# geonuklee/slam-toolkit

Measured on NVIDIA B200. Metric: orb_extract_match_stereo_frames_per_s, higher is better.
Workload: dtype u8

## Files before the change

slam-toolkit_b200/csrc/sfe_extract.cu:

```cuda
#include <cuda_fp16.h>

#include <algorithm>
#include <cmath>
#include <mutex>
#include <type_traits>

#include "sfe_extract.cuh"

namespace sfe {

__device__ __forceinline__ uint32_t ldg_word_at(const uint8_t *p) {
    const uintptr_t a = (uintptr_t)p;
    const uint32_t *w = (const uint32_t *)(a & ~(uintptr_t)3);
    return __funnelshift_r(__ldg(w), __ldg(w + 1), (uint32_t)(a & 3) * 8);
}

__device__ __forceinline__ uint32_t dp4a_u8u8(uint32_t a, uint32_t b, uint32_t c) {
    uint32_t d;
    asm("dp4a.u32.u32 %0, %1, %2, %3;" : "=r"(d) : "r"(a), "r"(b), "r"(c));
    return d;
}
__device__ __forceinline__ uint32_t dp2a_lo(uint32_t a, uint32_t b, uint32_t c) {
    uint32_t d;
    asm("dp2a.lo.u32.u32 %0, %1, %2, %3;" : "=r"(d) : "r"(a), "r"(b), "r"(c));
    return d;
}
__device__ __forceinline__ uint32_t dp2a_hi(uint32_t a, uint32_t b, uint32_t c) {
    uint32_t d;
    asm("dp2a.hi.u32.u32 %0, %1, %2, %3;" : "=r"(d) : "r"(a), "r"(b), "r"(c));
    return d;
}

__global__ void __launch_bounds__(256) realign_kernel(const uint8_t *__restrict__ src, size_t src_stride, int src_pitch,
                                                      uint8_t *__restrict__ dst, size_t dst_stride, int dst_pitch, int w, int h) {
    pdl_enter();
    const int x = (blockIdx.x * 32 + threadIdx.x) * 16, y = blockIdx.y * 8 + threadIdx.y, img = blockIdx.z;
    if (x >= dst_pitch || y >= h) return;
    const uint8_t *p = src + (size_t)img * src_stride + (size_t)y * src_pitch + x;
    uint4 v;
    if (x + 20 <= w) {
        v = make_uint4(ldg_word_at(p), ldg_word_at(p + 4), ldg_word_at(p + 8), ldg_word_at(p + 12));
    } else {
        uint32_t q[4] = {0, 0, 0, 0};
#pragma unroll
        for (int k = 0; k < 16; k++)
            if (x + k < w) q[k >> 2] |= (uint32_t)__ldg(p + k) << (8 * (k & 3));
        v = make_uint4(q[0], q[1], q[2], q[3]);
    }
    *(uint4 *)(dst + (size_t)img * dst_stride + (size_t)y * dst_pitch + x) = v;
}

constexpr int kPyrTileW = 64, kPyrTileH = 64;

struct PyrStep {
    int w, h, pitch, plane_off;
    int src_w, src_pitch, src_plane_off, src_is_input;
    int xtab_off, ytab_off;
    int src_level, box_w, box_h;
    int wide_h;
};

template <bool kTma>
__global__ void __launch_bounds__(256) pyr_resize_kernel(ImgSet S, PyrStep P, const uint2 *__restrict__ xtab,
                                                         const uint2 *__restrict__ ytab, const __grid_constant__ TmaMaps M) {
    pdl_enter();
    extern __shared__ __align__(128) uint8_t pyr_smem[];
    uint16_t *pyr_u = (uint16_t *)(pyr_smem + (kTma ? P.box_w * P.box_h : 0));
    __shared__ uint64_t bar;
    const int x0 = blockIdx.x * kPyrTileW, y0 = blockIdx.y * kPyrTileH, img = blockIdx.z, tid = threadIdx.x;
    const uint2 *yt = ytab + P.ytab_off;
    const int sy_first = __ldg(&yt[y0]).x & 0xFFFF;
    const int n_rows = (int)(__ldg(&yt[min(y0 + kPyrTileH, P.h) - 1]).x >> 16) - sy_first + 1;
    const int slot = slot_of(S, img);
    const int xa = (int)__ldg(&xtab[P.xtab_off + x0]).x & ~15;
    if (kTma && tid == 0) {
        mbar_init(&bar, 1);
        mbar_expect_tx(&bar, (uint32_t)(P.box_w * P.box_h));
        const bool set_a = img < S.split;
        const CUtensorMap *map = P.src_is_input ? (set_a ? &M.lv[0] : &M.l0b) : &M.lv[P.src_level];
        const int z = P.src_is_input ? S.in_z0 + (set_a ? img : img - S.split) : slot;
        tma_load_3d(pyr_smem, map, &bar, xa, sy_first, z);
    }
    {
        const int ox = tid & (kPyrTileW - 1);
        const uint2 xt = __ldg(&xtab[P.xtab_off + min(x0 + ox, P.w - 1)]);
        const int sx = xt.x, d1 = min(sx + 1, P.src_w - 1) - sx;
        const uint32_t w0 = xt.y & 0xFFFF, w1 = xt.y >> 16;
        if (kTma && P.wide_h) {
            const int g4 = (tid & 15) * 4, gi = P.xtab_off + min(x0 + g4, (P.w - 1) & ~3);
            const uint4 ta = __ldg((const uint4 *)&xtab[gi]), tb = __ldg((const uint4 *)&xtab[gi + 2]);
            const int o0 = (int)ta.x - xa;
            const uint32_t sh8 = (uint32_t)(o0 & 3) * 8;
            const uint32_t r1 = ta.z - ta.x, r2 = tb.x - ta.x, r3 = tb.z - ta.x;
            const uint32_t s0 = 0x10u, s1 = r1 | (r1 + 1) << 4, s2 = r2 | (r2 + 1) << 4, s3 = r3 | (r3 + 1) << 4;
            __syncthreads();
            mbar_wait(&bar, 0);
            const uint32_t *p = (const uint32_t *)pyr_smem + (tid >> 4) * (P.box_w >> 2) + (o0 >> 2);
            const int step = 16 * (P.box_w >> 2);
            for (int r = tid >> 4; r < n_rows; r += 16) {
                const uint32_t a = __funnelshift_r(p[0], p[1], sh8), b = __funnelshift_r(p[1], p[2], sh8);
                const uint32_t u0 = dp2a_lo(ta.y, __byte_perm(a, b, s0), 0) >> 4, u1 = dp2a_lo(ta.w, __byte_perm(a, b, s1), 0) >> 4;
                const uint32_t u2 = dp2a_lo(tb.y, __byte_perm(a, b, s2), 0) >> 4, u3 = dp2a_lo(tb.w, __byte_perm(a, b, s3), 0) >> 4;
                *(uint2 *)&pyr_u[r * kPyrTileW + g4] = make_uint2(u0 | u1 << 16, u2 | u3 << 16);
                p += step;
            }
        } else if (kTma) {
            __syncthreads();
            mbar_wait(&bar, 0);
            const uint8_t *p = pyr_smem + (tid >> 6) * P.box_w + (sx - xa);
            const int step = 4 * P.box_w;
            for (int r = tid >> 6; r < n_rows; r += 4) {
                pyr_u[r * kPyrTileW + ox] = (uint16_t)((p[0] * w0 + p[d1] * w1) >> 4);
                p += step;
            }
        } else {
            const uint8_t *src;
            if (P.src_is_input)
                src = img < S.split ? S.in_a + (size_t)img * S.in_stride : S.in_b + (size_t)(img - S.split) * S.in_stride;
            else
                src = S.pyr + (size_t)slot * S.pyr_stride + P.src_plane_off;
            const uint8_t *p = src + (size_t)(sy_first + (tid >> 6)) * P.src_pitch + sx;
            const int step = 4 * P.src_pitch;
            for (int r = tid >> 6; r < n_rows; r += 4) {
                pyr_u[r * kPyrTileW + ox] = (uint16_t)((__ldg(p) * w0 + __ldg(p + d1) * w1) >> 4);
                p += step;
            }
        }
    }
    __syncthreads();
    const int cg = (tid & 15) * 4, ry = tid >> 4;
    if (x0 + cg >= P.w) return;
    uint8_t *dst = S.pyr + (size_t)slot * S.pyr_stride + P.plane_off + x0 + cg;
#pragma unroll
    for (int k = 0; k < kPyrTileH / 16; k++) {
        const int oy = y0 + ry + 16 * k;
        if (oy >= P.h) break;
        const uint2 t = __ldg(&yt[oy]);
        const int r0 = (int)(t.x & 0xFFFF) - sy_first, r1 = (int)(t.x >> 16) - sy_first;
        const uint32_t b0 = t.y << 16, b1 = t.y & 0xFFFF0000u;
        const uint2 A = *(const uint2 *)&pyr_u[r0 * kPyrTileW + cg], B = *(const uint2 *)&pyr_u[r1 * kPyrTileW + cg];
        const uint32_t a[4] = {A.x & 0xFFFF, A.x >> 16, A.y & 0xFFFF, A.y >> 16};
        const uint32_t b[4] = {B.x & 0xFFFF, B.x >> 16, B.y & 0xFFFF, B.y >> 16};
        uint32_t v[4];
#pragma unroll
        for (int i = 0; i < 4; i++) v[i] = (__umulhi(b0, a[i]) + __umulhi(b1, b[i]) + 2) >> 2;
        *(uint32_t *)(dst + (size_t)oy * P.pitch) = v[0] | v[1] << 8 | v[2] << 16 | v[3] << 24;
    }
}


template <int TP>
__device__ __forceinline__ void fast_best_x2(const uint8_t *c0, const uint8_t *c1, int &best0, int &best1) {
    constexpr int off[16] = {3 * TP,  3 * TP + 1,  2 * TP + 2,  TP + 3,  3,  -TP + 3, -2 * TP + 2, -3 * TP + 1,
                             -3 * TP, -3 * TP - 1, -2 * TP - 2, -TP - 3, -3, TP - 3,  2 * TP - 2,  3 * TP - 1};
    uint32_t p[16], lo3[16], hi3[16];
#pragma unroll
    for (int k = 0; k < 16; k++) p[k] = __byte_perm(c0[off[k]], c1[off[k]], 0x5410);
#pragma unroll
    for (int s = 0; s < 16; s++) {
        lo3[s] = __vimin3_s16x2(p[s], p[(s + 1) & 15], p[(s + 2) & 15]);
        hi3[s] = __vimax3_s16x2(p[s], p[(s + 1) & 15], p[(s + 2) & 15]);
    }
    uint32_t max_of_min = 0u, min_of_max = 0x7fff7fffu;
#pragma unroll
    for (int s = 0; s < 16; s += 2) {
        const uint32_t l0 = __vimin3_s16x2(lo3[s], lo3[(s + 3) & 15], lo3[(s + 6) & 15]);
        const uint32_t l1 = __vimin3_s16x2(lo3[s + 1], lo3[(s + 4) & 15], lo3[(s + 7) & 15]);
        const uint32_t h0 = __vimax3_s16x2(hi3[s], hi3[(s + 3) & 15], hi3[(s + 6) & 15]);
        const uint32_t h1 = __vimax3_s16x2(hi3[s + 1], hi3[(s + 4) & 15], hi3[(s + 7) & 15]);
        max_of_min = __vimax3_s16x2(max_of_min, l0, l1);
        min_of_max = __vimin3_s16x2(min_of_max, h0, h1);
    }
    const int v0 = c0[0], v1 = c1[0];
    best0 = max(v0 - (int)(min_of_max & 0xFFFF), (int)(max_of_min & 0xFFFF) - v0);
    best1 = max(v1 - (int)(min_of_max >> 16), (int)(max_of_min >> 16) - v1);
}

template <bool kTma>
__global__ void __launch_bounds__(kFastThreads, kFastCtasPerSm) fast_segments_kernel(ImgSet S, FastPlan P, const SegRec *__restrict__ segs,
                                                                     const __grid_constant__ TmaMaps M) {
    constexpr int TP = kFastTilePitch, TW = TP / 4, SP = kFastScorePitch, T = kFastThreads;
    pdl_enter();
    extern __shared__ __align__(128) uint32_t fast_smem[];
    uint32_t *tile32 = fast_smem;
    uint8_t *score = (uint8_t *)(tile32 + P.tile_rows * TW);
    uint16_t *pre = (uint16_t *)(score + P.score_rows * SP);
    uint16_t *det = pre + P.list_cap;
    __shared__ int n_pre, n_det;
    __shared__ int cell_surv[kFastMaxCells];
    __shared__ uint64_t bar;
    const uint8_t *tile = (const uint8_t *)tile32;

    const uint4 rec = __ldg((const uint4 *)segs + blockIdx.x);
    const int ini_x = (short)(rec.x & 0xFFFF), ini_y = (short)(rec.x >> 16), tw = (short)(rec.y & 0xFFFF);
    const int sh = (rec.y >> 16) & 0xFF, level = rec.y >> 24, n_cells = rec.z & 0xFF, w_cell = (rec.z >> 8) & 0xFF;
    const int inv_w = rec.z >> 16, th = sh - 6;
    const FastLevel &F = P.lv[level];
    const int img = blockIdx.y, tid = threadIdx.x, lane = tid & 31, warp = tid >> 5;
    const int xa = (ini_x - 4) & ~15;
// ... 821 lines not shown
    if (y < 0) a = __fsub_rn(360.f, a);
    return a;
}

constexpr int kUmax[16] = {15, 15, 15, 15, 14, 14, 14, 13, 13, 12, 11, 10, 9, 8, 6, 3};
constexpr bool disc_is_symmetric() {
    for (int u = 0; u < 16; u++)
        for (int v = 0; v < 16; v++)
            if ((u <= kUmax[v]) != (v <= kUmax[u])) return false;
    return true;
}
static_assert(disc_is_symmetric(), "IC_Angle disc must be symmetric");
struct DiscTable {
    uint32_t u[16][8], in[16][8];
};
constexpr DiscTable make_disc_table() {
    DiscTable t{};
    for (int v = 0; v < 16; v++)
        for (int j = 0; j < 8; j++)
            for (int k = 0; k < 4; k++) {
                const int u = -kHalfPatch + 4 * j + k, au = u < 0 ? -u : u;
                if (au <= kUmax[v]) {
                    t.u[v][j] |= (uint32_t)(u & 0xFF) << (8 * k);
                    t.in[v][j] |= 1u << (8 * k);
                }
            }
    return t;
}
__device__ const DiscTable g_disc = make_disc_table();

__device__ __forceinline__ int dp4a_u8s8(uint32_t pix, uint32_t w, int acc) {
    int d;
    asm("dp4a.u32.s32 %0, %1, %2, %3;" : "=r"(d) : "r"(pix), "r"(w), "r"(acc));
    return d;
}

constexpr int kPatchR = 18;
constexpr int kPatchRows = 2 * kPatchR + 1, kPatchWords = 10;
constexpr signed char kPatternHost[1024] = {
#include "orb_pattern_data.inc"
};
constexpr bool pattern_within_patch() {
    for (int i = 0; i < 512; i++) {
        const int px = kPatternHost[2 * i], py = kPatternHost[2 * i + 1];
        if (4 * (px * px + py * py) >= (2 * kPatchR + 1) * (2 * kPatchR + 1)) return false;
    }
    return true;
}
static_assert(pattern_within_patch(), "a rotated pattern point could round outside the staged window");
#ifndef SFE_KP_PER_WARP
#define SFE_KP_PER_WARP 8
#endif
constexpr int kKpPerWarp = SFE_KP_PER_WARP;

constexpr int kIcBoxW = 48, kIcBoxH = 2 * kHalfPatch + 1, kBdBoxW = 64, kBdBoxH = kPatchRows;
constexpr int kIcBytes = 1536, kWinBytes = kIcBytes + 2432;
struct OrientMaps {
    CUtensorMap ic[kMaxLevels], ic_l0b;
    CUtensorMap bd[kMaxLevels];
};

template <bool kTma>
__global__ void __launch_bounds__(256, 5) orient_describe_kernel(ImgSet S, OutSet O, int kp_per_warp, const __grid_constant__ OrientMaps M) {
    __shared__ float2 pat[16 * 32];
    __shared__ __align__(128) uint8_t win_all[8][kTma ? kWinBytes : kPatchRows * kPatchWords * 4];
    __shared__ uint64_t bars[8];
    pdl_enter();
    const int tid = threadIdx.x, lane = tid & 31, warp = tid >> 5, img = blockIdx.y, slot = slot_of(S, img);
    uint32_t *patch = (uint32_t *)win_all[warp];
    uint32_t phase = 0;
    if (kTma && lane == 0) mbar_init(&bars[warp], 1);
    for (int i = tid; i < 512; i += 256) {
        const int byte = i >> 4, s = i & 15;
        pat[s * 32 + byte] = make_float2((float)g_pattern[2 * i], (float)g_pattern[2 * i + 1]);
    }
    const int wj = lane & 7, wr0 = 2 * (lane >> 3);
    auto ic_row = [wr0](int t) { return 8 * (t >> 1) + (t & 1) + wr0; };
    uint32_t wu[8], win[8];
#pragma unroll
    for (int t = 0; t < 8; t++) {
        const int r = ic_row(t), adv = r < 31 ? (r < kHalfPatch ? kHalfPatch - r : r - kHalfPatch) : 0;
        wu[t] = r < 31 ? __ldg(&g_disc.u[adv][wj]) : 0u;
        win[t] = r < 31 ? __ldg(&g_disc.in[adv][wj]) : 0u;
    }
    __syncthreads();
    const int cnt = lane < S.nlevels ? min(S.kp_count[slot * S.nlevels + lane], S.lv[lane].kp_cap) : 0;
    int inc = cnt;
#pragma unroll
    for (int o = 1; o < kMaxLevels; o <<= 1) {
        const int u = __shfl_up_sync(0xffffffffu, inc, o);
        if (lane >= o) inc += u;
    }
    const int total = __shfl_sync(0xffffffffu, inc, kMaxLevels - 1);
    const bool set_a = img < S.split;
    const int oi = set_a ? img : img - S.split;
    if (blockIdx.x == 0 && tid == 0) {
        (set_a ? O.n_a : O.n_b)[oi] = min(total, O.cap);
        if (total > O.cap) atomicOr(&S.flags[slot], kFlagOutOverflow);
    }
    const int g0 = (blockIdx.x * 8 + warp) * kp_per_warp;
    for (int g = g0; g < g0 + kp_per_warp; g++) {
        if (g >= total || g >= O.cap) return;
        const int l = __popc(__ballot_sync(0xffffffffu, lane < S.nlevels && inc <= g));
        const int local = g - __shfl_sync(0xffffffffu, inc - cnt, min(l, 31));
        const LevelPlan &L = S.lv[l];
        const uint32_t v = S.kpst[(size_t)slot * S.kpst_stride + L.kp_off + local];
        const int x = (v & 0xFFF) + kBorder, y = ((v >> 12) & 0xFFF) + kBorder;
        int pitch;
        const uint8_t *lvl = level_pixels(S, l, img, pitch);
        int m10 = 0, m01 = 0;
        const int xl = x - kPatchR, xb0 = xl & ~15;
        if (kTma) {
            const int xi = x - kHalfPatch, xi0 = xi & ~15;
            __syncwarp();
            if (lane == 0) {
                mbar_expect_tx(&bars[warp], kIcBoxW * kIcBoxH + kBdBoxW * kBdBoxH);
                const bool sa = img < S.split;
                const CUtensorMap *mi = l == 0 ? (sa ? &M.ic[0] : &M.ic_l0b) : &M.ic[l];
                tma_load_3d(win_all[warp], mi, &bars[warp], xi0, y - kHalfPatch, l == 0 ? S.in_z0 + (sa ? img : img - S.split) : slot);
                tma_load_3d(win_all[warp] + kIcBytes, &M.bd[l], &bars[warp], xb0, y - kPatchR, slot);
            }
            mbar_wait(&bars[warp], phase);
            phase ^= 1;
            const int o = xi - xi0;
            const uint32_t *w0 = (const uint32_t *)(win_all[warp] + (o & ~3) + 4 * wj);
            const uint32_t sh8 = (uint32_t)(o & 3) * 8;
#pragma unroll
            for (int t = 0; t < 8; t++) {
                const int r = ic_row(t);
                if (r < 31) {
                    const uint32_t *wp = w0 + r * (kIcBoxW / 4);
                    const uint32_t px = __funnelshift_r(wp[0], wp[1], sh8);
                    m10 = dp4a_u8s8(px, wu[t], m10);
                    m01 += (r - kHalfPatch) * dp4a_u8s8(px, win[t], 0);
                }
            }
        } else {
            const uint8_t *r0p = lvl + (size_t)(y - kHalfPatch) * pitch + (x - kHalfPatch + 4 * wj);
#pragma unroll
            for (int t = 0; t < 8; t++) {
                const int r = ic_row(t);
                if (r < 31) {
                    const uint8_t *rp = r0p + (size_t)r * pitch;
                    const uint32_t *wp = (const uint32_t *)((uintptr_t)rp & ~(uintptr_t)3);
                    const uint32_t px = __funnelshift_r(__ldg(wp), __ldg(wp + 1), ((uint32_t)(uintptr_t)rp & 3) * 8);
                    m10 = dp4a_u8s8(px, wu[t], m10);
                    m01 += (r - kHalfPatch) * dp4a_u8s8(px, win[t], 0);
                }
            }
        }
#pragma unroll
        for (int o = 16; o > 0; o >>= 1) {
            m01 += __shfl_xor_sync(0xffffffffu, m01, o);
            m10 += __shfl_xor_sync(0xffffffffu, m10, o);
        }
        const float angle = fast_atan2_deg((float)m01, (float)m10);
        float a = 0.f, b = 0.f;
        if (lane == 0) {
            const float factor_pi = (float)(3.1415926535897932384626433832795 / 180.0);
            const float rad = __fmul_rn(angle, factor_pi);
            double sn, cs;
            sincos((double)rad, &sn, &cs);
            a = (float)cs;
            b = (float)sn;
        }
        a = __shfl_sync(0xffffffffu, a, 0);
        b = __shfl_sync(0xffffffffu, b, 0);
        const uint8_t *pc;
        int wpitch;
        if (kTma) {
            wpitch = kBdBoxW;
            pc = win_all[warp] + kIcBytes + kPatchR * kBdBoxW + (xl - xb0) + kPatchR;
        } else {
            const int bp = L.blur_pitch;
            const uint8_t *bl = S.blur + (size_t)slot * S.blur_stride + L.blur_off;
            const int al = xl & 3;
            __syncwarp();
            if (lane < 3 * kPatchWords) {
                const int rs = lane / kPatchWords, c = lane - rs * kPatchWords;
                const uint32_t *src = (const uint32_t *)(bl + (size_t)(y - kPatchR + rs) * bp + (xl - al)) + c;
                uint32_t *dst = patch + rs * kPatchWords + c;
#pragma unroll
                for (int r = rs; r < kPatchRows; r += 3, src += 3 * (bp >> 2), dst += 3 * kPatchWords) *dst = __ldg(src);
            }
            __syncwarp();
            wpitch = kPatchWords * 4;
            pc = (const uint8_t *)patch + kPatchR * (kPatchWords * 4) + kPatchR + al;
        }
        uint32_t byte = 0;
#pragma unroll
        for (int k = 0; k < 8; k++) {
            int tv[2];
#pragma unroll
            for (int s = 0; s < 2; s++) {
                const float2 pp = pat[(2 * k + s) * 32 + lane];
                const int ry = __float2int_rn(__fadd_rn(__fmul_rn(pp.x, b), __fmul_rn(pp.y, a)));
                const int rx = __float2int_rn(__fsub_rn(__fmul_rn(pp.x, a), __fmul_rn(pp.y, b)));
                tv[s] = pc[ry * wpitch + rx];
            }
            byte |= (uint32_t)(tv[0] < tv[1]) << k;
        }
        uint8_t *desc = (set_a ? O.desc_a : O.desc_b) + ((size_t)oi * O.cap + g) * 32;
        desc[lane] = (uint8_t)byte;
        if (lane == 0) {
            sfe_keypoint kp;
            kp.x = (float)x;
            kp.y = (float)y;
            if (l != 0) {
                kp.x = __fmul_rn(kp.x, L.scale);
                kp.y = __fmul_rn(kp.y, L.scale);
            }
            kp.size = L.size;
            kp.angle = angle;
            kp.response = (float)(v >> 24);
            kp.octave = l;
            kp.class_id = -1;
            (set_a ? O.kps_a : O.kps_b)[(size_t)oi * O.cap + g] = kp;
        }
    }
}

}

using namespace sfe;

enum { kStagePyramid, kStageFast, kStageQuadtree, kStageBlur, kStageDescribe, kStageStereo, kStageTrack, kNumStages };
constexpr int kOctreeSmemCand = 3072;
constexpr int kComputeStreams = 4;
constexpr int kMaxChunks = 16;

struct sfe_extractor {
    int device = 0;
    cudaStream_t stream = nullptr;
    cudaStream_t s_h2d = nullptr, s_d2h = nullptr;
    cudaStream_t extra[kComputeStreams - 1] = {};
    int n_compute = 3;
    cudaStream_t aux[3] = {nullptr, nullptr, nullptr};
    cudaEvent_t ev_fork[3] = {}, ev_join[3] = {};
    int dev_split = 3;
    bool split_small = false;
    int octree_ctas = 0;
    int sm_count = 148;
    bool piped_now = false;
    bool orient_tma = true;
    bool overlap_tail = true;
    bool tail_pending = false;
    int overlap_blur = 2;
    cudaEvent_t ev_start = nullptr;
    bool async_dev = false;
    cudaEvent_t ev_in[kMaxChunks] = {}, ev_done[kMaxChunks] = {};
    int chunks_override = 0;
    bool trace = false;
    cudaEvent_t tr_ev[3 * kMaxChunks + 1] = {};
    sfe_extractor_params prm{};
    float scale[kMaxLevels], inv_scale[kMaxLevels], sigma2[kMaxLevels], inv_sigma2[kMaxLevels];
    int quota[kMaxLevels];
    int max_images = 0;
    int w = 0, h = 0;
    LevelPlan lv[kMaxLevels];
    FastPlan fast{};
    alignas(64) TmaMaps fast_maps{}, blur_maps{}, pyr_maps{};
    alignas(64) OrientMaps orient_maps{};
    int pyr_box_w = 0, pyr_box_h = 0;
    bool tma_plan_ok = false, tma_disabled = false, tma_now = false;
    const void *l0_key[2] = {nullptr, nullptr};
    size_t l0_geom[4] = {0, 0, 0, 0};
    int pitch0 = 0;
    std::vector<SegRec> segs;
    int seg_level_start[kMaxLevels + 1] = {};
    DevBuf<SegRec> d_segs;
    size_t fast_smem = 0, pyr_smem = 0;
    int pyr_wide_h[kMaxLevels] = {};
    std::vector<TilePlan> tiles;
    size_t pyr_stride = 0, blur_stride = 0;
    int cand_stride = 0, kpst_stride = 0, max_cand = 0, max_nodes = 0;
    size_t octree_smem = 0;
    int octree_smem_cand = 0, octree_slots = 0, octree_cand_override = 0;
    struct GraphEntry {
        uint64_t plan_gen = 0;
        int frames = 0, cap = 0, stereo = 0, seen = 0;
        double sp[3] = {0, 0, 0};
        const void *ptr[7] = {};
        cudaGraphExec_t exec = nullptr;
        int64_t launches = 0;
        uint64_t used = 0;
    };
    std::vector<GraphEntry> graphs;
    uint64_t plan_gen = 0, graph_clock = 0;
    bool use_graphs = true;
    bool use_pdl = true;
    bool octree_ff = true;
    bool pdl_now = false;
    bool octree_wide = false;
    int cand_floor[kMaxLevels] = {};
    int cand_cap_override = 0;
    DevBuf<uint8_t> d_octree_scratch;
    DevBuf<uint8_t> d_pyr, d_blur, d_in, d_l0, d_desc;
    DevBuf<uint32_t> d_cand, d_kpst;
    DevBuf<int> d_counts;
    DevBuf<TilePlan> d_tiles;
    DevBuf<uint2> d_xtab, d_ytab;
    DevBuf<sfe_keypoint> d_kps;
    DevBuf<int32_t> d_nout, d_sidx, d_sdist, d_tidx, d_tdist;
    std::vector<int> h_flags;
    int *h_flags_pinned = nullptr;
    uint8_t *h_stage = nullptr;
    size_t h_stage_bytes = 0;
    bool use_copy_kernel = true;
    int64_t launches = 0;
    bool profiling = false;
    cudaEvent_t prof_ev[kNumStages + 1] = {};
    bool prof_pending = false, prof_has_stereo = false, prof_has_track = false;
    TrackScratch track;
    double stage_ms[kNumStages] = {};
    int64_t stage_calls = 0;
    ImgSet last{};
    int last_count = 0;
};

static inline int cv_round_f(float v) { return (int)nearbyintf(v); }

static inline void prof_mark(sfe_extractor *ex, int i) {
    if (ex->profiling) cudaEventRecord(ex->prof_ev[i], ex->stream);
}

static void build_tables(sfe_extractor *ex) {
    const int nl = ex->prm.nlevels;
    const double sf = (double)ex->prm.scale_factor;
    ex->scale[0] = 1.0f;
    ex->sigma2[0] = 1.0f;
    for (int i = 1; i < nl; i++) {
        ex->scale[i] = (float)((double)ex->scale[i - 1] * sf);
        ex->sigma2[i] = ex->scale[i] * ex->scale[i];
    }
    for (int i = 0; i < nl; i++) {
        ex->inv_scale[i] = 1.0f / ex->scale[i];
        ex->inv_sigma2[i] = 1.0f / ex->sigma2[i];
    }
    const float factor = (float)(1.0 / sf);
    const float denom = 1 - (float)pow((double)factor, (double)nl);
    float want = (float)ex->prm.nfeatures * (1 - factor) / denom;
    int sum = 0;
    for (int l = 0; l < nl - 1; l++) {
        ex->quota[l] = cv_round_f(want);
        sum += ex->quota[l];
        want *= factor;
    }
    ex->quota[nl - 1] = std::max(ex->prm.nfeatures - sum, 0);
}

static void drop_graphs(sfe_extractor *ex) {
    for (auto &g : ex->graphs)
        if (g.exec) cudaGraphExecDestroy(g.exec);
    ex->graphs.clear();
}

static int build_plan(sfe_extractor *ex, int w, int h) {
    const int nl = ex->prm.nlevels;
    drop_graphs(ex);
    ex->plan_gen++;
    std::vector<uint2> xtab, ytab;
    int max_src_rows = 1, max_src_cols = 1;
    memset(&ex->fast, 0, sizeof(ex->fast));
    ex->segs.clear();
    int max_sh = 7, max_list = 8;
    ex->tiles.clear();
    size_t pyr_off = 0, blur_off = 0;
    int cand_off = 0, kp_off = 0, max_cand = 0, max_nodes = 8;
    for (int l = 0; l < nl; l++) {
        LevelPlan &L = ex->lv[l];
        memset(&L, 0, sizeof(L));
        L.w = cv_round_f((float)w * ex->inv_scale[l]);
        L.h = cv_round_f((float)h * ex->inv_scale[l]);
        SFE_REQUIRE(L.w >= 1 && L.h >= 1, SFE_ERR_UNSUPPORTED, "pyramid level collapses to zero size");
        SFE_REQUIRE(L.w <= 4096 + 2 * kBorder && L.h <= 4096 + 2 * kBorder, SFE_ERR_UNSUPPORTED,
                    "image larger than 4128 px per side");
        L.pitch = (int)align_up((size_t)L.w, 16);
        L.blur_pitch = L.pitch;
        if (l > 0) {
            L.plane_off = (int)pyr_off;
            pyr_off += align_up((size_t)L.pitch * L.h, 128);
        }
        L.blur_off = (int)blur_off;
        blur_off += align_up((size_t)L.blur_pitch * L.h, 128);
        L.scale = ex->scale[l];
        L.size = (float)(int)(31 * ex->scale[l]);
        L.quota = ex->quota[l];
        const int max_bx = L.w - kBorder, max_by = L.h - kBorder;
        L.win_w = max_bx - kBorder;
        L.win_h = max_by - kBorder;
        const float width = (float)L.win_w, height = (float)L.win_h;
        L.n_cols = L.win_w > 0 ? (int)(width / 30.f) : 0;
        L.n_rows = L.win_h > 0 ? (int)(height / 30.f) : 0;
        L.w_cell = L.h_cell = 1;
        int tested = 0, n_level_cells = 0;
        if (L.n_cols >= 1 && L.n_rows >= 1) {
            L.w_cell = (int)ceilf(width / L.n_cols);
            L.h_cell = (int)ceilf(height / L.n_rows);
            int rows_eff = 0, cols_eff = 0;
            for (int i = 0; i < L.n_rows; i++)
                if (kBorder + i * L.h_cell < max_by - 3 && max_by - (kBorder + i * L.h_cell) >= 7) rows_eff = i + 1;
            for (int j = 0; j < L.n_cols; j++)
                if (kBorder + j * L.w_cell < max_bx - 6) cols_eff = j + 1;
            SFE_REQUIRE(L.w_cell + 6 <= kMaxSub && L.h_cell + 6 <= kMaxSub, SFE_ERR_UNSUPPORTED, "FAST cell larger than 66 px");
            if (rows_eff > 0 && cols_eff > 0) {
                FastLevel &F = ex->fast.lv[l];
                F.pitch = L.pitch;
                F.plane_off = L.plane_off;
                n_level_cells = rows_eff * cols_eff;
                const int inv_w = 65536 / L.w_cell + 1;
                for (int x = 0; x < 256; x++) SFE_REQUIRE(((x * inv_w) >> 16) == x / L.w_cell && inv_w < 65536, SFE_ERR_UNSUPPORTED, "cell reciprocal");
                for (int i = 0; i < rows_eff; i++) {
                    const int ini_y = kBorder + i * L.h_cell, sh = std::min(ini_y + L.h_cell + 6, max_by) - ini_y;
                    max_sh = std::max(max_sh, sh);
                    for (int j = 0; j < cols_eff;) {
// ... 24 lines not shown
            L.n_ini = (int)roundf((float)L.win_w / (float)L.win_h);
            SFE_REQUIRE(L.n_ini >= 1, SFE_ERR_UNSUPPORTED,
                        "portrait level (W/H < 0.5): the reference divides by nIni == 0");
            L.hx = (float)L.win_w / (float)L.n_ini;
        }
        L.ff_depth = 0;
        while (ex->octree_ff && L.ff_depth < 6 && 4ll * L.n_ini * (1ll << (2 * (L.ff_depth + 1))) <= L.quota) L.ff_depth++;
        L.cand_cap = tested > 0 ? std::max(std::min(ex->cand_cap_override > 0 ? ex->cand_cap_override : std::max(tested / 12, 1024), kNarrowCandCap),
                                           std::min(ex->cand_floor[l], kMaxCandCap)) : 0;
        L.cand_off = cand_off;
        cand_off += L.cand_cap;
        ex->fast.lv[l].cand_off = L.cand_off;
        ex->fast.lv[l].cand_cap = L.cand_cap;
        L.kp_cap = tested > 0 ? std::max(L.quota + 3, 4 * L.n_ini) + 1 : 0;
        L.kp_off = kp_off;
        kp_off += L.kp_cap;
        max_cand = std::max(max_cand, L.cand_cap);
        max_nodes = std::max(max_nodes, std::max(L.kp_cap + 4, L.n_ini));
        if (tested > 0)
            for (int y0 = 0; y0 < L.h; y0 += kBlurTileH)
                for (int x0 = 0; x0 < L.w; x0 += kBlurTileW) ex->tiles.push_back(TilePlan{(short)l, (short)x0, (short)y0, 0});
        if (l > 0) {
            const int sw = ex->lv[l - 1].w, sh = ex->lv[l - 1].h;
            while (xtab.size() % 4) xtab.push_back(xtab.back());
            L.xtab_off = (int)xtab.size();
            L.ytab_off = (int)ytab.size();
            const double scale_x = 1.0 / ((double)L.w / sw), scale_y = 1.0 / ((double)L.h / sh);
            for (int dx = 0; dx < L.w; dx++) {
                float fx = (float)((dx + 0.5) * scale_x - 0.5);
                int sx = (int)floorf(fx);
                fx -= sx;
                if (sx < 0) { fx = 0; sx = 0; }
                if (sx >= sw - 1) { fx = 0; sx = sw - 1; }
                const int w0 = cv_round_f((1.f - fx) * 2048), w1 = cv_round_f(fx * 2048);
                xtab.push_back(make_uint2((unsigned)sx, (unsigned)w0 | (unsigned)w1 << 16));
            }
            while (xtab.size() % 4) xtab.push_back(xtab.back());
            ex->pyr_wide_h[l] = 1;
            for (int gx = 0; gx < L.w; gx += 4)
                if (xtab[L.xtab_off + gx + 3].x - xtab[L.xtab_off + gx].x > 6) ex->pyr_wide_h[l] = 0;
            for (int dy = 0; dy < L.h; dy++) {
                float fy = (float)((dy + 0.5) * scale_y - 0.5);
                int sy = (int)floorf(fy);
                fy -= sy;
                const int b0 = cv_round_f((1.f - fy) * 2048), b1 = cv_round_f(fy * 2048);
                const int y0 = std::min(std::max(sy, 0), sh - 1), y1 = std::min(std::max(sy + 1, 0), sh - 1);
                ytab.push_back(make_uint2((unsigned)y0 | (unsigned)y1 << 16, (unsigned)b0 | (unsigned)b1 << 16));
            }
            for (int tx = 0; tx < L.w; tx += kPyrTileW) {
                const int last = std::min(tx + kPyrTileW, L.w) - 1;
                const int first_sx = (int)xtab[L.xtab_off + tx].x & ~15;
                max_src_cols = std::max(max_src_cols, std::min((int)xtab[L.xtab_off + last].x + 1, sw - 1) - first_sx + 1);
            }
            for (int ty = 0; ty < L.h; ty += kPyrTileH) {
                const int last = std::min(ty + kPyrTileH, L.h) - 1;
                const int span = (int)(ytab[L.ytab_off + last].x >> 16) - (int)(ytab[L.ytab_off + ty].x & 0xFFFF) + 1;
                max_src_rows = std::max(max_src_rows, span);
            }
        }
    }
    ex->pyr_stride = std::max<size_t>(pyr_off, 128);
    ex->blur_stride = std::max<size_t>(blur_off, 128);
    ex->cand_stride = std::max(cand_off, 1);
    ex->kpst_stride = std::max(kp_off, 1);
    ex->max_cand = (std::max(max_cand, 1) + 7) & ~7;
    ex->max_nodes = max_nodes;
    ex->pyr_smem = (size_t)max_src_rows * kPyrTileW * sizeof(uint16_t);
    ex->pyr_box_w = (int)align_up((size_t)max_src_cols, 16);
    ex->pyr_box_h = max_src_rows;
    SFE_REQUIRE(ex->pyr_smem + (size_t)ex->pyr_box_w * ex->pyr_box_h <= 48 * 1024 && ex->pyr_box_w <= 256 && ex->pyr_box_h <= 256,
                SFE_ERR_UNSUPPORTED, "scale factor too large for the pyramid tile");
    ex->fast.nlevels = nl;
    ex->fast.ini_th = ex->prm.ini_th_fast;
    ex->fast.min_th = ex->prm.min_th_fast;
    ex->fast.n_segs = (int)ex->segs.size();
    ex->fast.tile_rows = (max_sh + 1) & ~1;
    ex->fast.score_rows = max_sh - 4;
    ex->fast.list_cap = (max_list + 7) & ~7;
    ex->fast_smem = (size_t)ex->fast.tile_rows * kFastTilePitch + (size_t)ex->fast.score_rows * kFastScorePitch + 2 * 2 * (size_t)ex->fast.list_cap;
    SFE_REQUIRE(ex->fast_smem <= 200 * 1024, SFE_ERR_UNSUPPORTED, "FAST segment working set exceeds shared memory");
    ex->octree_smem_cand = std::min(ex->max_cand, ex->octree_cand_override > 0 ? ex->octree_cand_override : kOctreeSmemCand) & ~7;
    if (ex->octree_smem_cand < 8) ex->octree_smem_cand = 8;
    ex->octree_wide = ex->max_cand > kNarrowCandCap;
    const size_t oct_cand_bytes = ex->octree_wide ? 16 : 14, oct_node_bytes = ex->octree_wide ? sizeof(ONodeT<true>) : sizeof(ONodeT<false>);
    ex->octree_smem = (size_t)ex->octree_smem_cand * oct_cand_bytes + (size_t)max_nodes * (16 + 3 * 4 + 2 * oct_node_bytes + 2 * 2 + 8) + 32 * 4 + 64;
    SFE_REQUIRE(ex->octree_smem <= 227 * 1024, SFE_ERR_UNSUPPORTED, "quadtree working set exceeds shared memory");
    {
        int big_levels = 0;
        for (int l = 0; l < nl; l++) big_levels += ex->lv[l].cand_cap > ex->octree_smem_cand;
        ex->octree_slots = big_levels * ex->max_images;
    }
    SFE_CUDA(ex->d_octree_scratch.ensure(std::max<size_t>((size_t)ex->octree_slots * ex->max_cand * oct_cand_bytes, 16)));
    const int n = ex->max_images;
    SFE_CUDA(ex->d_pyr.ensure(ex->pyr_stride * n));
    SFE_CUDA(ex->d_blur.ensure(ex->blur_stride * n));
    SFE_CUDA(ex->d_cand.ensure((size_t)ex->cand_stride * n));
    SFE_CUDA(ex->d_kpst.ensure((size_t)ex->kpst_stride * n));
    SFE_CUDA(ex->d_counts.ensure((size_t)n * (2 * nl + 1) + 1));
    SFE_CUDA(cudaMemsetAsync(ex->d_counts.p, 0, sizeof(int) * ex->d_counts.n, ex->stream));
    SFE_CUDA(ex->d_tiles.ensure(std::max<size_t>(ex->tiles.size(), 1)));
    SFE_CUDA(ex->d_segs.ensure(std::max<size_t>(ex->segs.size(), 1)));
    if (!ex->segs.empty())
        SFE_CUDA(cudaMemcpyAsync(ex->d_segs.p, ex->segs.data(), sizeof(SegRec) * ex->segs.size(), cudaMemcpyHostToDevice, ex->stream));
    SFE_CUDA(ex->d_xtab.ensure(std::max<size_t>(xtab.size(), 1)));
    SFE_CUDA(ex->d_ytab.ensure(std::max<size_t>(ytab.size(), 1)));
    if (!ex->tiles.empty())
        SFE_CUDA(cudaMemcpyAsync(ex->d_tiles.p, ex->tiles.data(), sizeof(TilePlan) * ex->tiles.size(), cudaMemcpyHostToDevice, ex->stream));
    if (!xtab.empty()) {
        SFE_CUDA(cudaMemcpyAsync(ex->d_xtab.p, xtab.data(), sizeof(uint2) * xtab.size(), cudaMemcpyHostToDevice, ex->stream));
        SFE_CUDA(cudaMemcpyAsync(ex->d_ytab.p, ytab.data(), sizeof(uint2) * ytab.size(), cudaMemcpyHostToDevice, ex->stream));
    }
    SFE_CUDA(cudaStreamSynchronize(ex->stream));
    ex->tma_plan_ok = !ex->tma_disabled;
    for (int l = 0; l < nl && ex->tma_plan_ok; l++) {
        const LevelPlan &L = ex->lv[l];
        if (L.w < 8 || L.h < 8) ex->tma_plan_ok = false;
        if (l == 0 || !ex->tma_plan_ok) continue;
        ex->tma_plan_ok = tma_encode_u8_3d(&ex->fast_maps.lv[l], ex->d_pyr.p + L.plane_off, L.w, L.h, n, L.pitch, ex->pyr_stride,
                                           kFastTilePitch, ex->fast.tile_rows) &&
                          tma_encode_u8_3d(&ex->blur_maps.lv[l], ex->d_pyr.p + L.plane_off, L.w, L.h, n, L.pitch, ex->pyr_stride,
                                           kBlurInWords * 4, kBlurTileH + 6) &&
                          (nl < 2 || tma_encode_u8_3d(&ex->pyr_maps.lv[l], ex->d_pyr.p + L.plane_off, L.w, L.h, n, L.pitch, ex->pyr_stride,
                                                      ex->pyr_box_w, ex->pyr_box_h)) &&
// ... 110 lines not shown
        if (!ok) return;
    }
    ex->tma_now = true;
}

constexpr bool kFastTma = true;

static int launch_fast(sfe_extractor *ex, cudaStream_t st, const ImgSet &S, int count, int level0 = 0, int level1 = kMaxLevels) {
    level1 = std::min(level1, ex->prm.nlevels);
    const int seg0 = ex->seg_level_start[level0], nseg = ex->seg_level_start[level1] - seg0;
    if (nseg <= 0) return SFE_OK;
    const dim3 grid((unsigned)nseg, count);
    if (ex->fast_smem > 48 * 1024) {
        static std::mutex mu;
        static size_t granted[64] = {};
        std::lock_guard<std::mutex> lock(mu);
        if (ex->fast_smem > granted[ex->device & 63]) {
            SFE_CUDA(cudaFuncSetAttribute(fast_segments_kernel<true>, cudaFuncAttributeMaxDynamicSharedMemorySize, (int)ex->fast_smem));
            SFE_CUDA(cudaFuncSetAttribute(fast_segments_kernel<false>, cudaFuncAttributeMaxDynamicSharedMemorySize, (int)ex->fast_smem));
            granted[ex->device & 63] = ex->fast_smem;
        }
    }
    {
        static std::once_flag once[64];
        std::call_once(once[ex->device & 63], [] {
            cudaFuncSetAttribute(fast_segments_kernel<true>, cudaFuncAttributePreferredSharedMemoryCarveout, cudaSharedmemCarveoutMaxShared);
            cudaFuncSetAttribute(fast_segments_kernel<false>, cudaFuncAttributePreferredSharedMemoryCarveout, cudaSharedmemCarveoutMaxShared);
        });
    }
    if (ex->tma_now && kFastTma)
        launch_k(fast_segments_kernel<true>, grid, kFastThreads, ex->fast_smem, st, ex->pdl_now, S, ex->fast, ex->d_segs.p + seg0, ex->fast_maps);
    else
        launch_k(fast_segments_kernel<false>, grid, kFastThreads, ex->fast_smem, st, ex->pdl_now, S, ex->fast, ex->d_segs.p + seg0, ex->fast_maps);
    return SFE_OK;
}

constexpr int kSplitMaxImages = 4;

static int join_tail(sfe_extractor *ex) {
    if (ex->tail_pending) {
        SFE_CUDA(cudaStreamWaitEvent(ex->stream, ex->ev_join[1], 0));
        ex->tail_pending = false;
    }
    return SFE_OK;
}

static int enqueue_extract(sfe_extractor *ex, cudaStream_t st, const ImgSet &S, int count, const OutSet &O) {
    const int nl = ex->prm.nlevels;
    prof_mark(ex, 0);
    auto launch_pyr = [&](int l) {
        const LevelPlan &D = ex->lv[l], &Q = ex->lv[l - 1];
        const PyrStep P{D.w, D.h, D.pitch, D.plane_off, Q.w, l == 1 ? S.in_pitch : Q.pitch, Q.plane_off, l == 1, D.xtab_off, D.ytab_off,
                        l - 1, ex->pyr_box_w, ex->pyr_box_h, ex->pyr_wide_h[l]};
        dim3 grid(div_up(D.w, kPyrTileW), div_up(D.h, kPyrTileH), count);
        if (ex->tma_now)
            launch_k(pyr_resize_kernel<true>, grid, 256, ex->pyr_smem + (size_t)ex->pyr_box_w * ex->pyr_box_h, st, ex->pdl_now, S, P, ex->d_xtab.p,
                     ex->d_ytab.p, ex->pyr_maps);
        else
            launch_k(pyr_resize_kernel<false>, grid, 256, ex->pyr_smem, st, ex->pdl_now, S, P, ex->d_xtab.p, ex->d_ytab.p, ex->pyr_maps);
        ex->launches++;
    };
    const bool has_cells = ex->fast.n_cells > 0;
    {
        static std::once_flag once[64];
        std::call_once(once[ex->device & 63], [] {
            const void *fns[] = {(const void *)pyr_resize_kernel<true>, (const void *)pyr_resize_kernel<false>, (const void *)blur_kernel<true>,
                                 (const void *)blur_kernel<false>, (const void *)octree_kernel<true>, (const void *)octree_kernel<false>,
                                 (const void *)orient_describe_kernel<true>, (const void *)orient_describe_kernel<false>,
                                 (const void *)realign_kernel};
            for (const void *f : fns) cudaFuncSetAttribute(f, cudaFuncAttributePreferredSharedMemoryCarveout, cudaSharedmemCarveoutMaxShared);
        });
    }
    if (has_cells) {
        static std::mutex mu;
        static size_t granted[64] = {};
        std::lock_guard<std::mutex> lock(mu);
        if (ex->octree_smem > granted[ex->device & 63]) {
            SFE_CUDA(cudaFuncSetAttribute(octree_kernel<false>, cudaFuncAttributeMaxDynamicSharedMemorySize, (int)ex->octree_smem));
            SFE_CUDA(cudaFuncSetAttribute(octree_kernel<true>, cudaFuncAttributeMaxDynamicSharedMemorySize, (int)ex->octree_smem));
            granted[ex->device & 63] = ex->octree_smem;
        }
    }
    int *scratch_next = ex->d_counts.p + (size_t)ex->max_images * nl * 2;
    auto launch_octree = [&](cudaStream_t so, int level0, int level_n, int ctas) {
        const int items = level_n * count;
        const int grid = ctas > 0 ? std::min(items, ctas) : items;
        const int threads = nl * count <= ex->sm_count / 2 ? 1024 : 256;
        if (ex->octree_wide)
            launch_k(octree_kernel<true>, grid, threads, ex->octree_smem, so, ex->pdl_now, S, count, level0, level_n, ex->octree_smem_cand,
                     ex->max_cand, ex->max_nodes, ex->d_octree_scratch.p, ex->octree_slots, scratch_next);
        else
            launch_k(octree_kernel<false>, grid, threads, ex->octree_smem, so, ex->pdl_now, S, count, level0, level_n, ex->octree_smem_cand,
                     ex->max_cand, ex->max_nodes, ex->d_octree_scratch.p, ex->octree_slots, scratch_next);
        ex->launches++;
    };
    const bool fork_ok = !ex->profiling && !ex->piped_now && st == ex->stream;
    const bool split = fork_ok && has_cells && ex->split_small && count <= kSplitMaxImages && nl >= 3;
    if (split) {
        launch_pyr(1);
        cudaStream_t sa = ex->aux[2];
        SFE_CUDA(cudaEventRecord(ex->ev_fork[2], st));
        SFE_CUDA(cudaStreamWaitEvent(sa, ex->ev_fork[2], 0));
        if (int rc = launch_fast(ex, sa, S, count, 0, 2)) return rc;
        launch_octree(sa, 0, 2, 0);
        SFE_CUDA(cudaEventRecord(ex->ev_join[2], sa));
        for (int l = 2; l < nl; l++) launch_pyr(l);
        cudaStream_t sb = ex->aux[0];
        SFE_CUDA(cudaEventRecord(ex->ev_fork[0], st));
        SFE_CUDA(cudaStreamWaitEvent(sb, ex->ev_fork[0], 0));
        if (ex->tma_now)
            blur_kernel<true><<<dim3((unsigned)ex->tiles.size(), count), 256, 0, sb>>>(S, ex->d_tiles.p, ex->blur_maps);
        else
            blur_kernel<false><<<dim3((unsigned)ex->tiles.size(), count), 256, 0, sb>>>(S, ex->d_tiles.p, ex->blur_maps);
        SFE_CUDA(cudaEventRecord(ex->ev_join[0], sb));
        if (int rc = launch_fast(ex, st, S, count, 2, nl)) return rc;
        launch_octree(st, 2, nl - 2, 0);
        SFE_CUDA(cudaStreamWaitEvent(st, ex->ev_join[2], 0));
        SFE_CUDA(cudaStreamWaitEvent(st, ex->ev_join[0], 0));
        ex->launches += 3;
// ... 921 lines not shown
```

Baseline: 68200.

## Add tall pyramid tiles, precomputed row table, and batched keypoint decode in describe

The pyramid resize kernel is templated on tile height. Large levels get 128-row tiles loaded with two TMA boxes, and a per-block shared table of vertical taps. The intermediate buffer widens to 32 bits, so the vertical pass packs results with byte_perm instead of per-element unpacking. Separately, orient_describe now has each lane decode one keypoint of the warp's run up front, uses a magic-number float rounding trick for pattern addressing, and writes keypoint structs in parallel across lanes rather than from lane 0 each iteration. These changes cut per-keypoint serial overhead and redundant loads, but raise shared memory per block, which may reduce occupancy.

New measurement: 69410, median of 6. +1.8%, better.

```diff
diff --git a/slam-toolkit_b200/csrc/sfe_extract.cu b/slam-toolkit_b200/csrc/sfe_extract.cu
--- a/slam-toolkit_b200/csrc/sfe_extract.cu
+++ b/slam-toolkit_b200/csrc/sfe_extract.cu
@@ -50,7 +50,9 @@
     *(uint4 *)(dst + (size_t)img * dst_stride + (size_t)y * dst_pitch + x) = v;
 }
 
-constexpr int kPyrTileW = 64, kPyrTileH = 64;
+constexpr int kPyrTileW = 64, kPyrTileH = 64, kPyrTallTileH = 128;
+constexpr int kPyrTallMinCtasPerSm = 4;
+constexpr size_t kPyrSmemMax = 200 * 1024;
 
 struct PyrStep {
     int w, h, pitch, plane_off;
@@ -60,26 +62,36 @@
     int wide_h;
 };
 
-template <bool kTma>
+template <bool kTma, int kTileH>
 __global__ void __launch_bounds__(256) pyr_resize_kernel(ImgSet S, PyrStep P, const uint2 *__restrict__ xtab,
                                                          const uint2 *__restrict__ ytab, const __grid_constant__ TmaMaps M) {
+    static_assert(kTileH % kPyrTileH == 0 && kTileH <= 256, "tile height: whole boxes, one table entry per thread");
+    constexpr int kBoxes = kTileH / kPyrTileH;
     pdl_enter();
     extern __shared__ __align__(128) uint8_t pyr_smem[];
-    uint16_t *pyr_u = (uint16_t *)(pyr_smem + (kTma ? P.box_w * P.box_h : 0));
+    uint32_t *pyr_u = (uint32_t *)(pyr_smem + (kTma ? kBoxes * P.box_w * P.box_h : 0));
+    __shared__ uint4 vrow[kTileH];
     __shared__ uint64_t bar;
-    const int x0 = blockIdx.x * kPyrTileW, y0 = blockIdx.y * kPyrTileH, img = blockIdx.z, tid = threadIdx.x;
+    const int x0 = blockIdx.x * kPyrTileW, y0 = blockIdx.y * kTileH, img = blockIdx.z, tid = threadIdx.x;
     const uint2 *yt = ytab + P.ytab_off;
     const int sy_first = __ldg(&yt[y0]).x & 0xFFFF;
-    const int n_rows = (int)(__ldg(&yt[min(y0 + kPyrTileH, P.h) - 1]).x >> 16) - sy_first + 1;
+    const int n_rows = (int)(__ldg(&yt[min(y0 + kTileH, P.h) - 1]).x >> 16) - sy_first + 1;
     const int slot = slot_of(S, img);
     const int xa = (int)__ldg(&xtab[P.xtab_off + x0]).x & ~15;
     if (kTma && tid == 0) {
         mbar_init(&bar, 1);
-        mbar_expect_tx(&bar, (uint32_t)(P.box_w * P.box_h));
+        const int boxes = kBoxes > 1 && n_rows > P.box_h ? 2 : 1;
+        mbar_expect_tx(&bar, (uint32_t)(boxes * P.box_w * P.box_h));
         const bool set_a = img < S.split;
         const CUtensorMap *map = P.src_is_input ? (set_a ? &M.lv[0] : &M.l0b) : &M.lv[P.src_level];
         const int z = P.src_is_input ? S.in_z0 + (set_a ? img : img - S.split) : slot;
         tma_load_3d(pyr_smem, map, &bar, xa, sy_first, z);
+        if (boxes > 1) tma_load_3d(pyr_smem + P.box_w * P.box_h, map, &bar, xa, sy_first + P.box_h, z);
+    }
+    if (tid < kTileH) {
+        const uint2 t = __ldg(&yt[min(y0 + tid, P.h - 1)]);
+        vrow[tid] = make_uint4(((t.x & 0xFFFF) - sy_first) * (kPyrTileW * 4), ((t.x >> 16) - sy_first) * (kPyrTileW * 4), t.y << 16,
+                               t.y & 0xFFFF0000u);
     }
     {
         const int ox = tid & (kPyrTileW - 1);
@@ -99,9 +111,9 @@
             const int step = 16 * (P.box_w >> 2);
             for (int r = tid >> 4; r < n_rows; r += 16) {
                 const uint32_t a = __funnelshift_r(p[0], p[1], sh8), b = __funnelshift_r(p[1], p[2], sh8);
-                const uint32_t u0 = dp2a_lo(ta.y, __byte_perm(a, b, s0), 0) >> 4, u1 = dp2a_lo(ta.w, __byte_perm(a, b, s1), 0) >> 4;
-                const uint32_t u2 = dp2a_lo(tb.y, __byte_perm(a, b, s2), 0) >> 4, u3 = dp2a_lo(tb.w, __byte_perm(a, b, s3), 0) >> 4;
-                *(uint2 *)&pyr_u[r * kPyrTileW + g4] = make_uint2(u0 | u1 << 16, u2 | u3 << 16);
+                *(uint4 *)&pyr_u[r * kPyrTileW + g4] =
+                    make_uint4(dp2a_lo(ta.y, __byte_perm(a, b, s0), 0) >> 4, dp2a_lo(ta.w, __byte_perm(a, b, s1), 0) >> 4,
+                               dp2a_lo(tb.y, __byte_perm(a, b, s2), 0) >> 4, dp2a_lo(tb.w, __byte_perm(a, b, s3), 0) >> 4);
                 p += step;
             }
         } else if (kTma) {
@@ -110,7 +122,7 @@
             const uint8_t *p = pyr_smem + (tid >> 6) * P.box_w + (sx - xa);
             const int step = 4 * P.box_w;
             for (int r = tid >> 6; r < n_rows; r += 4) {
-                pyr_u[r * kPyrTileW + ox] = (uint16_t)((p[0] * w0 + p[d1] * w1) >> 4);
+                pyr_u[r * kPyrTileW + ox] = (p[0] * w0 + p[d1] * w1) >> 4;
                 p += step;
             }
         } else {
@@ -122,7 +134,7 @@
             const uint8_t *p = src + (size_t)(sy_first + (tid >> 6)) * P.src_pitch + sx;
             const int step = 4 * P.src_pitch;
             for (int r = tid >> 6; r < n_rows; r += 4) {
-                pyr_u[r * kPyrTileW + ox] = (uint16_t)((__ldg(p) * w0 + __ldg(p + d1) * w1) >> 4);
+                pyr_u[r * kPyrTileW + ox] = (__ldg(p) * w0 + __ldg(p + d1) * w1) >> 4;
                 p += step;
             }
         }
@@ -130,21 +142,19 @@
     __syncthreads();
     const int cg = (tid & 15) * 4, ry = tid >> 4;
     if (x0 + cg >= P.w) return;
-    uint8_t *dst = S.pyr + (size_t)slot * S.pyr_stride + P.plane_off + x0 + cg;
+    uint8_t *dst = S.pyr + (size_t)slot * S.pyr_stride + P.plane_off + (size_t)(y0 + ry) * P.pitch + x0 + cg;
+    const uint8_t *ucol = (const uint8_t *)(pyr_u + cg);
+    const int rows_left = P.h - y0 - ry;
 #pragma unroll
-    for (int k = 0; k < kPyrTileH / 16; k++) {
-        const int oy = y0 + ry + 16 * k;
-        if (oy >= P.h) break;
-        const uint2 t = __ldg(&yt[oy]);
-        const int r0 = (int)(t.x & 0xFFFF) - sy_first, r1 = (int)(t.x >> 16) - sy_first;
-        const uint32_t b0 = t.y << 16, b1 = t.y & 0xFFFF0000u;
-        const uint2 A = *(const uint2 *)&pyr_u[r0 * kPyrTileW + cg], B = *(const uint2 *)&pyr_u[r1 * kPyrTileW + cg];
-        const uint32_t a[4] = {A.x & 0xFFFF, A.x >> 16, A.y & 0xFFFF, A.y >> 16};
-        const uint32_t b[4] = {B.x & 0xFFFF, B.x >> 16, B.y & 0xFFFF, B.y >> 16};
-        uint32_t v[4];
-#pragma unroll
-        for (int i = 0; i < 4; i++) v[i] = (__umulhi(b0, a[i]) + __umulhi(b1, b[i]) + 2) >> 2;
-        *(uint32_t *)(dst + (size_t)oy * P.pitch) = v[0] | v[1] << 8 | v[2] << 16 | v[3] << 24;
+    for (int k = 0; k < kTileH / 16; k++) {
+        if (16 * k >= rows_left) break;
+        const uint4 t = vrow[ry + 16 * k];
+        const uint4 A = *(const uint4 *)(ucol + t.x), B = *(const uint4 *)(ucol + t.y);
+        const uint32_t e = __byte_perm(__umulhi(t.z, A.x), __umulhi(t.z, A.z), 0x5410) + __byte_perm(__umulhi(t.w, B.x), __umulhi(t.w, B.z), 0x5410) +
+                           0x00020002u;
+        const uint32_t o = __byte_perm(__umulhi(t.z, A.y), __umulhi(t.z, A.w), 0x5410) + __byte_perm(__umulhi(t.w, B.y), __umulhi(t.w, B.w), 0x5410) +
+                           0x00020002u;
+        *(uint32_t *)(dst + (size_t)(16 * k) * P.pitch) = ((e >> 2) & 0x00FF00FFu) | ((o << 6) & 0xFF00FF00u);
     }
 }
 
@@ -1072,6 +1082,10 @@
 #define SFE_KP_PER_WARP 8
 #endif
 constexpr int kKpPerWarp = SFE_KP_PER_WARP;
+static_assert(kKpPerWarp >= 1 && kKpPerWarp <= 32, "lane k of a warp decodes keypoint k of its run");
+
+constexpr float kRoundMagic = 12582912.f;
+constexpr uint32_t kRoundBias = 0x4B400000u;
 
 constexpr int kIcBoxW = 48, kIcBoxH = 2 * kHalfPatch + 1, kBdBoxW = 64, kBdBoxH = kPatchRows;
 constexpr int kIcBytes = 1536, kWinBytes = kIcBytes + 2432;
@@ -1085,6 +1099,8 @@
     __shared__ float2 pat[16 * 32];
     __shared__ __align__(128) uint8_t win_all[8][kTma ? kWinBytes : kPatchRows * kPatchWords * 4];
     __shared__ uint64_t bars[8];
+    __shared__ uint2 run_kp[8][32];
+    __shared__ float run_angle[8][32];
     pdl_enter();
     const int tid = threadIdx.x, lane = tid & 31, warp = tid >> 5, img = blockIdx.y, slot = slot_of(S, img);
     uint32_t *patch = (uint32_t *)win_all[warp];
@@ -1119,13 +1135,22 @@
         if (total > O.cap) atomicOr(&S.flags[slot], kFlagOutOverflow);
     }
     const int g0 = (blockIdx.x * 8 + warp) * kp_per_warp;
-    for (int g = g0; g < g0 + kp_per_warp; g++) {
-        if (g >= total || g >= O.cap) return;
-        const int l = __popc(__ballot_sync(0xffffffffu, lane < S.nlevels && inc <= g));
-        const int local = g - __shfl_sync(0xffffffffu, inc - cnt, min(l, 31));
+    const int n = min(min(total, O.cap) - g0, kp_per_warp);
+    if (n <= 0) return;
+    {
+        const int g = g0 + lane;
+        int l = 0;
+        for (int j = 0; j < S.nlevels - 1; j++) l += __shfl_sync(0xffffffffu, inc, j) <= g;
+        const int first = __shfl_sync(0xffffffffu, inc - cnt, l);
+        if (lane < n) run_kp[warp][lane] = make_uint2(S.kpst[(size_t)slot * S.kpst_stride + S.lv[l].kp_off + (g - first)], (uint32_t)l);
+        __syncwarp();
+    }
+    for (int k = 0; k < n; k++) {
+        const int g = g0 + k;
+        const uint2 e = run_kp[warp][k];
+        const int l = e.y;
         const LevelPlan &L = S.lv[l];
-        const uint32_t v = S.kpst[(size_t)slot * S.kpst_stride + L.kp_off + local];
-        const int x = (v & 0xFFF) + kBorder, y = ((v >> 12) & 0xFFF) + kBorder;
+        const int x = (e.x & 0xFFF) + kBorder, y = ((e.x >> 12) & 0xFFF) + kBorder;
         int pitch;
         const uint8_t *lvl = level_pixels(S, l, img, pitch);
         int m10 = 0, m01 = 0;
@@ -1186,6 +1211,7 @@
         }
         a = __shfl_sync(0xffffffffu, a, 0);
         b = __shfl_sync(0xffffffffu, b, 0);
+        if (lane == 0) run_angle[warp][k] = angle;
         const uint8_t *pc;
         int wpitch;
         if (kTma) {
@@ -1207,36 +1233,41 @@
             wpitch = kPatchWords * 4;
             pc = (const uint8_t *)patch + kPatchR * (kPatchWords * 4) + kPatchR + al;
         }
+        const uint32_t unbias = 0u - kRoundBias * (uint32_t)(wpitch + 1);
         uint32_t byte = 0;
 #pragma unroll
-        for (int k = 0; k < 8; k++) {
+        for (int k8 = 0; k8 < 8; k8++) {
             int tv[2];
 #pragma unroll
             for (int s = 0; s < 2; s++) {
-                const float2 pp = pat[(2 * k + s) * 32 + lane];
-                const int ry = __float2int_rn(__fadd_rn(__fmul_rn(pp.x, b), __fmul_rn(pp.y, a)));
-                const int rx = __float2int_rn(__fsub_rn(__fmul_rn(pp.x, a), __fmul_rn(pp.y, b)));
-                tv[s] = pc[ry * wpitch + rx];
-            }
-            byte |= (uint32_t)(tv[0] < tv[1]) << k;
+                const float2 pp = pat[(2 * k8 + s) * 32 + lane];
+                const uint32_t ry = __float_as_uint(__fadd_rn(__fadd_rn(__fmul_rn(pp.x, b), __fmul_rn(pp.y, a)), kRoundMagic));
+                const uint32_t rx = __float_as_uint(__fadd_rn(__fsub_rn(__fmul_rn(pp.x, a), __fmul_rn(pp.y, b)), kRoundMagic));
+                tv[s] = pc[(int)(ry * (uint32_t)wpitch + rx + unbias)];
+            }
+            byte |= (uint32_t)(tv[0] < tv[1]) << k8;
         }
         uint8_t *desc = (set_a ? O.desc_a : O.desc_b) + ((size_t)oi * O.cap + g) * 32;
         desc[lane] = (uint8_t)byte;
-        if (lane == 0) {
-            sfe_keypoint kp;
-            kp.x = (float)x;
-            kp.y = (float)y;
-            if (l != 0) {
-                kp.x = __fmul_rn(kp.x, L.scale);
-                kp.y = __fmul_rn(kp.y, L.scale);
-            }
-            kp.size = L.size;
-            kp.angle = angle;
-            kp.response = (float)(v >> 24);
-            kp.octave = l;
-            kp.class_id = -1;
-            (set_a ? O.kps_a : O.kps_b)[(size_t)oi * O.cap + g] = kp;
-        }
+    }
+    __syncwarp();
+    if (lane < n) {
+        const uint2 e = run_kp[warp][lane];
+        const int l = e.y;
+        const LevelPlan &L = S.lv[l];
+        sfe_keypoint kp;
+        kp.x = (float)((e.x & 0xFFF) + kBorder);
+        kp.y = (float)(((e.x >> 12) & 0xFFF) + kBorder);
+        if (l != 0) {
+            kp.x = __fmul_rn(kp.x, L.scale);
+            kp.y = __fmul_rn(kp.y, L.scale);
+        }
+        kp.size = L.size;
+        kp.angle = run_angle[warp][lane];
+        kp.response = (float)(e.x >> 24);
+        kp.octave = l;
+        kp.class_id = -1;
+        (set_a ? O.kps_a : O.kps_b)[(size_t)oi * O.cap + g0 + lane] = kp;
     }
 }
 
@@ -1289,7 +1320,7 @@
     std::vector<SegRec> segs;
     int seg_level_start[kMaxLevels + 1] = {};
     DevBuf<SegRec> d_segs;
-    size_t fast_smem = 0, pyr_smem = 0;
+    size_t fast_smem = 0, pyr_smem = 0, pyr_smem_tall = 0;
     int pyr_wide_h[kMaxLevels] = {};
     std::vector<TilePlan> tiles;
     size_t pyr_stride = 0, blur_stride = 0;
@@ -1380,7 +1411,7 @@
     drop_graphs(ex);
     ex->plan_gen++;
     std::vector<uint2> xtab, ytab;
-    int max_src_rows = 1, max_src_cols = 1;
+    int max_src_rows = 1, max_src_rows_tall = 1, max_src_cols = 1;
     memset(&ex->fast, 0, sizeof(ex->fast));
     ex->segs.clear();
     int max_sh = 7, max_list = 8;
@@ -1511,11 +1542,16 @@
                 const int first_sx = (int)xtab[L.xtab_off + tx].x & ~15;
                 max_src_cols = std::max(max_src_cols, std::min((int)xtab[L.xtab_off + last].x + 1, sw - 1) - first_sx + 1);
             }
-            for (int ty = 0; ty < L.h; ty += kPyrTileH) {
-                const int last = std::min(ty + kPyrTileH, L.h) - 1;
-                const int span = (int)(ytab[L.ytab_off + last].x >> 16) - (int)(ytab[L.ytab_off + ty].x & 0xFFFF) + 1;
-                max_src_rows = std::max(max_src_rows, span);
-            }
+            auto src_rows = [&](int tile_h) {
+                int rows = 1;
+                for (int ty = 0; ty < L.h; ty += tile_h) {
+                    const int last = std::min(ty + tile_h, L.h) - 1;
+                    rows = std::max(rows, (int)(ytab[L.ytab_off + last].x >> 16) - (int)(ytab[L.ytab_off + ty].x & 0xFFFF) + 1);
+                }
+                return rows;
+            };
+            max_src_rows = std::max(max_src_rows, src_rows(kPyrTileH));
+            max_src_rows_tall = std::max(max_src_rows_tall, src_rows(kPyrTallTileH));
         }
     }
     ex->pyr_stride = std::max<size_t>(pyr_off, 128);
@@ -1524,10 +1560,12 @@
     ex->kpst_stride = std::max(kp_off, 1);
     ex->max_cand = (std::max(max_cand, 1) + 7) & ~7;
     ex->max_nodes = max_nodes;
-    ex->pyr_smem = (size_t)max_src_rows * kPyrTileW * sizeof(uint16_t);
     ex->pyr_box_w = (int)align_up((size_t)max_src_cols, 16);
-    ex->pyr_box_h = max_src_rows;
-    SFE_REQUIRE(ex->pyr_smem + (size_t)ex->pyr_box_w * ex->pyr_box_h <= 48 * 1024 && ex->pyr_box_w <= 256 && ex->pyr_box_h <= 256,
+    ex->pyr_box_h = (int)align_up((size_t)max_src_rows, 8);
+    ex->pyr_smem = (size_t)max_src_rows * kPyrTileW * sizeof(uint32_t);
+    ex->pyr_smem_tall = (size_t)max_src_rows_tall * kPyrTileW * sizeof(uint32_t);
+    SFE_REQUIRE(max_src_rows_tall <= 2 * max_src_rows && ex->pyr_box_w <= 256 && ex->pyr_box_h <= 256 &&
+                    ex->pyr_smem_tall + 2 * (size_t)ex->pyr_box_w * ex->pyr_box_h <= kPyrSmemMax,
                 SFE_ERR_UNSUPPORTED, "scale factor too large for the pyramid tile");
     ex->fast.nlevels = nl;
     ex->fast.ini_th = ex->prm.ini_th_fast;
@@ -1744,19 +1782,32 @@
         const LevelPlan &D = ex->lv[l], &Q = ex->lv[l - 1];
         const PyrStep P{D.w, D.h, D.pitch, D.plane_off, Q.w, l == 1 ? S.in_pitch : Q.pitch, Q.plane_off, l == 1, D.xtab_off, D.ytab_off,
                         l - 1, ex->pyr_box_w, ex->pyr_box_h, ex->pyr_wide_h[l]};
-        dim3 grid(div_up(D.w, kPyrTileW), div_up(D.h, kPyrTileH), count);
-        if (ex->tma_now)
-            launch_k(pyr_resize_kernel<true>, grid, 256, ex->pyr_smem + (size_t)ex->pyr_box_w * ex->pyr_box_h, st, ex->pdl_now, S, P, ex->d_xtab.p,
+        const dim3 tall(div_up(D.w, kPyrTileW), div_up(D.h, kPyrTallTileH), count);
+        const bool use_tall = (size_t)tall.x * tall.y * tall.z >= (size_t)kPyrTallMinCtasPerSm * ex->sm_count;
+        const dim3 grid = use_tall ? tall : dim3(div_up(D.w, kPyrTileW), div_up(D.h, kPyrTileH), count);
+        const size_t box = (size_t)ex->pyr_box_w * ex->pyr_box_h;
+        if (ex->tma_now && use_tall)
+            launch_k(pyr_resize_kernel<true, kPyrTallTileH>, grid, 256, ex->pyr_smem_tall + 2 * box, st, ex->pdl_now, S, P, ex->d_xtab.p,
                      ex->d_ytab.p, ex->pyr_maps);
+        else if (ex->tma_now)
+            launch_k(pyr_resize_kernel<true, kPyrTileH>, grid, 256, ex->pyr_smem + box, st, ex->pdl_now, S, P, ex->d_xtab.p, ex->d_ytab.p,
+                     ex->pyr_maps);
+        else if (use_tall)
+            launch_k(pyr_resize_kernel<false, kPyrTallTileH>, grid, 256, ex->pyr_smem_tall, st, ex->pdl_now, S, P, ex->d_xtab.p, ex->d_ytab.p,
+                     ex->pyr_maps);
         else
-            launch_k(pyr_resize_kernel<false>, grid, 256, ex->pyr_smem, st, ex->pdl_now, S, P, ex->d_xtab.p, ex->d_ytab.p, ex->pyr_maps);
+            launch_k(pyr_resize_kernel<false, kPyrTileH>, grid, 256, ex->pyr_smem, st, ex->pdl_now, S, P, ex->d_xtab.p, ex->d_ytab.p,
+                     ex->pyr_maps);
         ex->launches++;
     };
     const bool has_cells = ex->fast.n_cells > 0;
     {
         static std::once_flag once[64];
         std::call_once(once[ex->device & 63], [] {
-            const void *fns[] = {(const void *)pyr_resize_kernel<true>, (const void *)pyr_resize_kernel<false>, (const void *)blur_kernel<true>,
+            const void *pyr[] = {(const void *)pyr_resize_kernel<true, kPyrTileH>, (const void *)pyr_resize_kernel<false, kPyrTileH>,
+                                 (const void *)pyr_resize_kernel<true, kPyrTallTileH>, (const void *)pyr_resize_kernel<false, kPyrTallTileH>};
+            for (const void *f : pyr) cudaFuncSetAttribute(f, cudaFuncAttributeMaxDynamicSharedMemorySize, (int)kPyrSmemMax);
+            const void *fns[] = {pyr[0], pyr[1], pyr[2], pyr[3], (const void *)blur_kernel<true>,
                                  (const void *)blur_kernel<false>, (const void *)octree_kernel<true>, (const void *)octree_kernel<false>,
                                  (const void *)orient_describe_kernel<true>, (const void *)orient_describe_kernel<false>,
                                  (const void *)realign_kernel};
```
